# atoms-ufrj/atomsmm

Hardware: AMD Instinct MI355X
Metric: ns/day on 100k-atom TIP3P RESPA box; near-nonbonded HBM GB/s vs 8 TB/s peak (higher is better)
Workload: dtype f64

## Files before the change

atomsmm_amd/csrc/abi.hip:

```cpp
#include <algorithm>
#include <cmath>
#include <cstring>
#include <numeric>

#include "amm_ctx.h"
#include "cluster.h"

int amm_pair_setup_grid(amm_ctx *ctx, PairForce *pf);
static bool amm_family_allows_cluster(int family, int flags) {
    const bool tab_family = family == AMM_NEAR_NONE || family == AMM_NEAR_SHIFT || family == AMM_NEAR_FSWITCH || family == AMM_DAMPED || family == AMM_NONBONDED;
    return tab_family && !(flags & (AMM_GROUP_LJ | AMM_GROUP_Q));
}
int amm_bonded_arity(int kind);
int amm_bonded_npar(int kind);

static thread_local std::string g_error;
void amm_set_error(const std::string &msg) { g_error = msg; }

static PairForce *get_pair(amm_ctx *ctx, int id) {
    if (!ctx || id < 0 || id >= (int)ctx->forces.size() || ctx->forces[id].type != AMM_FORCE_PAIR) {
        amm_set_error("invalid pair force id");
        return nullptr;
    }
    return ctx->forces[id].pair;
// ... 1222 lines not shown
            long long c2 = 0;
            if (amm_pair_count_within_impl(ctx, pf->rest, d_pos, r_within, &c2)) return 1;
            c += c2;
        }
    } else if (amm_pair_count_within_impl(ctx, pf, d_pos, r_within, &c)) return 1;
    *count = (int64_t)c;
    return 0;
}

const char *amm_kernel_revision(void) { return amm_kernel_revision_impl(); }

int amm_set_outer_skin(amm_ctx *ctx, double skin_out) {
    ctx->skin_out = skin_out;
    return 0;
}

int amm_set_option(amm_ctx *ctx, const char *name, double value) {
    if (!ctx || !name) {
        amm_set_error("amm_set_option: null argument");
        return 1;
    }
    const std::string k(name);
    const int v = (int)value;
    if (k == "cluster") ctx->opt_cluster = v;
    else if (k == "hybrid") ctx->opt_hybrid = v;
    else if (k == "small_group") ctx->opt_small_group = v;
    else if (k == "mixed_terms") ctx->opt_mixed_terms = v;
    else if (k == "rest_skin_factor") ctx->opt_rest_skin_factor = value;
    else if (k == "tab") ctx->opt_tab = v;
    else if (k == "site_trips") ctx->site_trips = v != 0;
    else if (k == "lanes_per_row") ctx->opt_lpa = v;
    else if (k == "build_parts") ctx->opt_parts = v;
    else if (k == "build_split") ctx->opt_build_split = v;
    else if (k == "unroll") ctx->opt_unroll = v;
    else if (k == "dual_unroll") ctx->opt_dual_unroll = v;
    else if (k == "tab_block") ctx->opt_tab_bs = v;
    else if (k == "tab_dual_block") ctx->opt_tab_dual_bs = v;
    else if (k == "fuse_rows") ctx->opt_fuse_rows = v;
    else if (k == "row_phases") ctx->opt_row_phases = v;
    else if (k == "group_candidates") ctx->opt_group_candidates = v;
    else if (k == "positions_private") ctx->opt_positions_private = v;
    else if (k == "site_tab") ctx->opt_site_tab = v;
    else if (k == "terms_from") ctx->opt_terms_from = v;
    else if (k == "no_term_lanes") ctx->opt_no_term_lanes = v;
    else if (k == "fuse_epilogue") ctx->opt_fuse_epilogue = v;
    else if (k == "comm_timeout") ctx->opt_comm_timeout = value;
    else if (k == "spec_assign") ctx->opt_spec_assign = v;
    else if (k == "chargeless") ctx->opt_chargeless = v;
    else if (k == "state_exchange") ctx->opt_state_exchange = v;
    else {
        amm_set_error("amm_set_option: unknown option '" + k + "'");
        return 1;
    }
    return 0;
}

static const double AMM_BOX_SKIN_KEEP = 0.5;
static const double AMM_BOX_ROWS_GROW = 1.25;

static double grid_room(const amm_ctx *ctx, const CellGrid &g) {
    double room = 1.0e30;
    for (int k = 0; k < 3; ++k) room = std::min(room, 2.0 * ctx->box.L[k] / g.nc[k]);
    return room;
}
static bool grid_differs(const amm_ctx *ctx, const CellGrid &g, double reach) {
    for (int k = 0; k < 3; ++k) {
// ... 228 lines not shown
```

atomsmm_amd/csrc/amm_ctx.h:

```cpp
#pragma once
#include <hip/hip_runtime.h>

#include <cstdint>
#include <string>
#include <vector>

#include "../../include/atomsmm_hip.h"

#define AMM_WAVE 64
#define AMM_MAX_PRE 6
#define AMM_DERIV_LAMBDA 1024
#define AMM_MAX_GROUPS 33

void amm_set_error(const std::string &msg);
#define AMM_HIP(call)                                                                            \
    do {                                                                                         \
        hipError_t e_ = (call);                                                                  \
        if (e_ != hipSuccess) {                                                                  \
            amm_set_error(std::string(#call) + ": " + hipGetErrorString(e_));                    \
            return 1;                                                                            \
        }                                                                                        \
    } while (0)

struct PairTab {
// ... 259 lines not shown
    BondedSet *bs = nullptr;
    double *f0 = nullptr;
    int npre = 0, niter = 0;
    const double *pre_a[AMM_MAX_PRE] = {nullptr}, *pre_b[AMM_MAX_PRE] = {nullptr};
    double pre_coef[AMM_MAX_PRE] = {0};
    int pre_plus[AMM_MAX_PRE] = {0};
    double c1 = 0, d = 0, c2 = 0;
    PairForce *next = nullptr;
    int kind = 0;
    int with_move = 0;
    double dcoef = 0;
};

struct amm_ctx {
    int n = 0;
    int opt_spec_assign = 1;
    int opt_state_exchange = 1;
    int opt_chargeless = 1;
    int opt_fuse_epilogue = 1;
    const EpiPlan *epi_request = nullptr;
    bool epi_done = false;
    long long n_epilogues = 0;
    long long n_state_exchanges = 0;
    std::vector<const double *> own_only;
    long long n_copies_current = 0;
    int opt_cluster = 1;
    int opt_hybrid = 1;
    double opt_rest_skin_factor = 2.0;
    int opt_mixed_terms = 1;
    int opt_small_group = 1;
    bool creating_rest = false;
    int opt_tab = 1;
    int opt_build_split = 0;
    int opt_lpa = 0, opt_parts = 0, opt_unroll = 2, opt_dual_unroll = 2, opt_tab_bs = 0, opt_tab_dual_bs = 0;
    int opt_site_tab = 1;
    CZeroRows zero_rows = CZeroRows{0, nullptr, nullptr, nullptr};
    int opt_positions_private = 0;
    int opt_group_candidates = 1;
    int opt_row_phases = 1;
    int opt_fuse_rows = 1;
    int opt_terms_from = 8192, opt_no_term_lanes = 0;
    ListWatch watched[AMM_MAX_WATCH];
    int n_watched = 0;
    int device = 0;
    hipStream_t stream = nullptr;
    Box box;
    bool has_box = true;
    int rank = 0, world = 1;
    std::vector<ForceObj> forces;
    double *d_x = nullptr, *d_v = nullptr;
    const double *d_mass = nullptr;
    double *slots[AMM_MAX_SLOTS] = {nullptr};
    GroupDef groups[AMM_MAX_GROUPS];
    bool profile = false;
    int profile_only = -1;
    double *d_scratch = nullptr;
    double *d_expr_part = nullptr;
    double *d_fscratch = nullptr;
    ConstraintSet *constraints = nullptr;
    std::vector<MinObj *> minimizers;
    std::vector<ExprDef> exprs;
    std::vector<BathDef> baths;
    IsoDef iso;
    RegDef reg;
    unsigned long long expr_seed = 0, expr_counter = 0;
    double *alt_x = nullptr, *alt_v = nullptr, *alt_f = nullptr;
// ... 120 lines not shown
```

atomsmm_amd/csrc/cluster.hip:

```cpp
#include <algorithm>
#include <cmath>
#include <cstdio>
#include <cstdlib>
#include <cstring>
#include <type_traits>
#include <vector>

#include "amm_ctx.h"
#include "bonded_terms.h"
#include "cluster.h"
#include "device_utils.h"
#include "pair_math.h"
#include "pair_tab.h"

#ifndef AMM_EXP_NOLJ
#define AMM_EXP_NOLJ 0
#endif

__device__ double amm_erfcx_table_dev_c[AMM_ERFCX_NI * AMM_ERFCX_NC];
static bool g_erfcx_uploaded_c[64] = {false};

void amm_cluster_classify(int n, const std::vector<int> &ptr, const std::vector<int> &idx, std::vector<int> &mol_first, std::vector<int> &rest) {
    mol_first.clear();
    rest.clear();
// ... 203 lines not shown
    for (int off = 32; off > 0; off >>= 1) {
        sum += __shfl_xor(sum, off);
        nr += __shfl_xor(nr, off);
        mx = max(mx, __shfl_xor(mx, off));
    }
    if ((threadIdx.x & 63) == 0) {
        sh_part[threadIdx.x >> 6][0] = sum;
        sh_part[threadIdx.x >> 6][1] = mx;
        sh_part[threadIdx.x >> 6][2] = nr;
    }
    __syncthreads();
    if (threadIdx.x == 0) {
        flags[2] = (int)max(max(sh_part[0][1], sh_part[1][1]), max(sh_part[2][1], sh_part[3][1]));
        counters[1] = sh_part[0][0] + sh_part[1][0] + sh_part[2][0] + sh_part[3][0];
        counters[2] = sh_part[0][2] + sh_part[1][2] + sh_part[2][2] + sh_part[3][2];
        if (!count_only) {
            flags[0] = 0;
            flags[AMM_FLAG_FAR] = 0;
            counters[0] += 1;
        }
    }
}

#ifndef CB_WAVES
#define CB_WAVES 5
#endif
#define CB_OCC __attribute__((amdgpu_waves_per_eu(CB_WAVES)))
#ifdef AMM_CBS_TIMING
__device__ unsigned long long g_cbs_t[8];
#define CBS_STAMP(i) do { const unsigned long long now_ = wall_clock64(); if (w == 0 && lane == 0) atomicAdd(&g_cbs_t[i], now_ - t_last); t_last = now_; } while (0)
#else
#define CBS_STAMP(i) do { } while (0)
#endif
template <bool COUNT_ONLY, bool RINT, bool SLICE = false>
__global__ void __launch_bounds__(256) __attribute__((amdgpu_waves_per_eu(SLICE ? 3 : CB_WAVES))) k_cbuild(int c_begin, int c_end, int parts, const int *__restrict__ cell_start,
                                                const float4 *__restrict__ pos4f, CBoxF box, CellGrid g, float rlist, float rnear2, int cap,
                                                int *nl, int *nnb, int *nnb_near, int *flags, unsigned long long *blockstats,
                                                unsigned long long *counters, int *ticket, int force, const int *slice_cells) {
    if (!force && !flags[0]) return;
    __shared__ int s_rstart[4][128];
    __shared__ int s_rpref[4][128];
    __shared__ float s_rshift[4][3][128];
    __shared__ int s_q[4][CB_BATCH][CB_QCAP];
    __shared__ unsigned char s_coarse[4][CB_COARSE];
    const int lane = threadIdx.x & 63, w = threadIdx.x >> 6;
    const int wave = __builtin_amdgcn_readfirstlane((int)((blockIdx.x * blockDim.x + threadIdx.x) >> 6));
    const float FAR = 1.0e9f;
    const float rlist2 = rlist * rlist;
    unsigned long long wsum = 0, wnear = 0;
    int wmax = 0;
    const int first_cell = SLICE ? __builtin_amdgcn_readfirstlane(slice_cells[0]) : 0;
    const int nunits = SLICE ? (__builtin_amdgcn_readfirstlane(slice_cells[1]) - first_cell + 1) * parts : g.ncell * parts;
    int unit = wave;
#ifdef AMM_CBS_TIMING
    unsigned long long t_last = wall_clock64(), t_drain = 0, n_drain = 0;
#endif
    do {
    const int c = unit < nunits ? first_cell + unit / parts : g.ncell, part = unit % parts;
    int a_begin = 0, a_end = 0;
    if (c < g.ncell) {
        const int cb0 = __builtin_amdgcn_readfirstlane(cell_start[c]), cb1 = __builtin_amdgcn_readfirstlane(cell_start[c + 1]);
        const int per = (cb1 - cb0 + parts - 1) / parts;
        a_begin = max(cb0 + part * per, c_begin);
        a_end = min(min(cb0 + (part + 1) * per, cb1), c_end);
    }
    if (a_begin < a_end) {
        const int ncx = g.nc[0], ncy = g.nc[1], ncz = g.nc[2];
        const int cx = c % ncx, cy = (c / ncx) % ncy, cz = c / (ncx * ncy);
        const int nsx = g.nstencil[0], nsy = g.nstencil[1], ne = nsx * nsy * g.nstencil[2];
        int total;
        {
            int ecs[2] = {0, 0}, len[2] = {0, 0}, inc[2];
            float esx[2] = {0.f, 0.f}, esy[2] = {0.f, 0.f}, esz[2] = {0.f, 0.f};
#pragma unroll
            for (int hh = 0; hh < 2; ++hh) {
                const int e = lane + 64 * hh;
                if (e < ne) {
                    const int ox = e % nsx, oy = (e / nsx) % nsy, oz = e / (nsx * nsy);
                    int nz = ncz < 2 * g.h[2] + 1 ? oz : cz - g.h[2] + oz;
                    esz[hh] = nz < 0 ? -box.L[2] : (nz >= ncz ? box.L[2] : 0.f);
                    nz = nz < 0 ? nz + ncz : (nz >= ncz ? nz - ncz : nz);
                    int ny = ncy < 2 * g.h[1] + 1 ? oy : cy - g.h[1] + oy;
                    esy[hh] = ny < 0 ? -box.L[1] : (ny >= ncy ? box.L[1] : 0.f);
                    ny = ny < 0 ? ny + ncy : (ny >= ncy ? ny - ncy : ny);
                    int nx = ncx < 2 * g.h[0] + 1 ? ox : cx - g.h[0] + ox;
                    esx[hh] = nx < 0 ? -box.L[0] : (nx >= ncx ? box.L[0] : 0.f);
                    nx = nx < 0 ? nx + ncx : (nx >= ncx ? nx - ncx : nx);
                    const int cc = (nz * ncy + ny) * ncx + nx;
                    ecs[hh] = cell_start[cc];
                    len[hh] = cell_start[cc + 1] - ecs[hh];
                }
                inc[hh] = len[hh];
                for (int off = 1; off < 64; off <<= 1) {
                    const int v = __shfl_up(inc[hh], off);
                    if (lane >= off) inc[hh] += v;
                }
            }
            const int lower = __builtin_amdgcn_readlane(inc[0], 63);
            total = lower + __builtin_amdgcn_readlane(inc[1], 63);
#pragma unroll
            for (int hh = 0; hh < 2; ++hh) {
                s_rstart[w][lane + 64 * hh] = ecs[hh];
                s_rpref[w][lane + 64 * hh] = (hh ? lower : 0) + inc[hh] - len[hh];
                s_rshift[w][0][lane + 64 * hh] = esx[hh];
                s_rshift[w][1][lane + 64 * hh] = esy[hh];
                s_rshift[w][2][lane + 64 * hh] = esz[hh];
            }
            __builtin_amdgcn_fence(__ATOMIC_RELEASE, "wavefront");
            __builtin_amdgcn_wave_barrier();
            __builtin_amdgcn_fence(__ATOMIC_ACQUIRE, "wavefront");
        }
        int cshift = 3;
        while (((total + 127) >> cshift) > CB_COARSE) ++cshift;
#pragma unroll
        for (int q = 0; q < CB_COARSE / 64; ++q) {
            const int idx = (lane + 64 * q) << cshift;
            int r = 0;
#pragma unroll
            for (int step = 64; step > 0; step >>= 1)
                if (s_rpref[w][r + step] <= idx) r += step;
            s_coarse[w][lane + 64 * q] = (unsigned char)r;
        }
        __builtin_amdgcn_fence(__ATOMIC_RELEASE, "wavefront");
        __builtin_amdgcn_wave_barrier();
        __builtin_amdgcn_fence(__ATOMIC_ACQUIRE, "wavefront");
#ifdef AMM_CBS_TIMING
        if (SLICE && lane == 0) { atomicAdd(&g_cbs_t[7], 1ull); atomicAdd(&g_cbs_t[0], wall_clock64() - t_last); }
#endif
        for (int tb = a_begin; tb < a_end; tb += CB_BATCH) {
            const int nt = min(CB_BATCH, a_end - tb);
            float4 my = make_float4(0.f, 0.f, 0.f, 0.f);
            if (lane < 3 * nt) my = pos4f[3 * tb + lane];
            int row_cnt = 0;
            int q_head = 0, q_cnt = 0;
            auto rl = [&](float v, int l) { return __int_as_float(__builtin_amdgcn_readlane(__float_as_int(v), l)); };
            auto drain = [&](int t, int n) {
#ifdef AMM_CBS_TIMING
                const unsigned long long t_d0 = wall_clock64();
                n_drain++;
#endif
                const int head = __builtin_amdgcn_readlane(q_head, t);
                int slot[2];
                bool v[2];
                float4 A[2][3];
#pragma unroll
                for (int u = 0; u < 2; ++u) {
                    const bool v0 = lane + 64 * u < n;
                    slot[u] = v0 ? s_q[w][t][cq_wrap(head + lane + 64 * u)] : tb + t;
                    v[u] = v0 && slot[u] != tb + t;
                }
#pragma unroll
                for (int u = 0; u < 2; ++u)
#pragma unroll
                    for (int b = 0; b < 3; ++b) A[u][b] = pos4f[3 * slot[u] + b];
                const int sites[2] = {__float_as_int(A[0][1].w), __float_as_int(A[1][1].w)};
                float px[3], py[3], pz[3];
#pragma unroll
                for (int a = 0; a < 3; ++a) {
                    px[a] = rl(my.x, 3 * t + a);
                    py[a] = rl(my.y, 3 * t + a);
                    pz[a] = rl(my.z, 3 * t + a);
                }
                v2f ax[3], ay[3], az[3];
#pragma unroll
                for (int b = 0; b < 3; ++b) {
                    ax[b] = v2f{A[0][b].x, A[1][b].x};
                    ay[b] = v2f{A[0][b].y, A[1][b].y};
                    az[b] = v2f{A[0][b].z, A[1][b].z};
                }
                if (!RINT) {
                    const v2f sx = box.L[0] * __builtin_elementwise_rint((ax[0] - px[0]) * box.invL[0]);
                    const v2f sy = box.L[1] * __builtin_elementwise_rint((ay[0] - py[0]) * box.invL[1]);
                    const v2f sz = box.L[2] * __builtin_elementwise_rint((az[0] - pz[0]) * box.invL[2]);
#pragma unroll
// ... 12 lines not shown
                        if (RINT) {
                            dx -= box.L[0] * __builtin_elementwise_rint(dx * box.invL[0]);
                            dy -= box.L[1] * __builtin_elementwise_rint(dy * box.invL[1]);
                            dz -= box.L[2] * __builtin_elementwise_rint(dz * box.invL[2]);
                        }
                        v2f r2 = dx * dx;
                        r2 = __builtin_elementwise_fma(dy, dy, r2);
                        r2 = __builtin_elementwise_fma(dz, dz, r2);
                        m2 = __builtin_elementwise_min(m2, r2);
                    }
#pragma unroll
                for (int u = 0; u < 2; ++u) {
                    const float m2u = u ? m2.y : m2.x;
                    const bool pass = v[u] && m2u < rlist2;
                    const unsigned long long m_pass = __builtin_amdgcn_ballot_w64(pass);
                    if (m_pass != 0ull) {
                        const bool is_near = pass && m2u < rnear2;
                        const unsigned long long m_near = __builtin_amdgcn_ballot_w64(is_near);
                        const int np_ = __popcll(m_pass), nn_ = __popcll(m_near);
                        const int c2 = __builtin_amdgcn_readlane(row_cnt, t);
                        const int cnt = c2 & 0xffff, cntf = (int)((unsigned)c2 >> 16);
                        if (!COUNT_ONLY) {
                            const int mp = __builtin_amdgcn_mbcnt_hi((unsigned)(m_pass >> 32), __builtin_amdgcn_mbcnt_lo((unsigned)m_pass, 0u));
                            const int mn = __builtin_amdgcn_mbcnt_hi((unsigned)(m_near >> 32), __builtin_amdgcn_mbcnt_lo((unsigned)m_near, 0u));
                            const int pos_near = cnt + mn, pos_far = (cap - 1 - cntf) - (mp - mn);
                            if (cnt + cntf + np_ <= cap) {
                                int *row_out = nl + (size_t)(tb + t - c_begin) * cap;
                                if (pass) row_out[is_near ? pos_near : pos_far] = slot[u] | (sites[u] << 29);
                            }
                        }
                        row_cnt = lane == t ? c2 + nn_ + ((np_ - nn_) << 16) : row_cnt;
                    }
                }
                q_head = lane == t ? cq_wrap(head + n) : q_head;
                q_cnt = lane == t ? q_cnt - n : q_cnt;
#ifdef AMM_CBS_TIMING
                t_drain += wall_clock64() - t_d0;
#endif
            };
            auto fetch = [&](int cb, float4 (&cand)[2], int (&js)[2]) {
#pragma unroll
                for (int u = 0; u < 2; ++u) {
                    const int idx = cb + u * 64 + lane;
                    const bool in = idx < total;
                    int r = s_coarse[w][idx >> cshift];
                    while (r < 127 && s_rpref[w][r + 1] <= idx) ++r;
                    const int slot = in ? s_rstart[w][r] + idx - s_rpref[w][r] : 0;
                    float4 q = pos4f[3 * slot];
                    if (!RINT) {
                        const float sx = s_rshift[w][0][r], sy = s_rshift[w][1][r], sz = s_rshift[w][2][r];
                        q.x = in ? q.x + sx : FAR;
                        q.y = in ? q.y + sy : FAR;
                        q.z = in ? q.z + sz : FAR;
                    } else if (!in) {
                        q.w = -1.0e9f;
                    }
                    cand[u] = q;
                    js[u] = slot;
                }
            };
            float4 cand[2], cand_n[2];
            int js[2], js_n[2];
            fetch(0, cand, js);
            const float plim_l = my.w + rlist;
            for (int cb = 0; cb < total; cb += 128) {
                if (cb + 128 < total) fetch(cb + 128, cand_n, js_n);
                const v2f cx = v2f{cand[0].x, cand[1].x}, cy = v2f{cand[0].y, cand[1].y}, cz = v2f{cand[0].z, cand[1].z};
                const v2f cw = v2f{cand[0].w, cand[1].w};
                for (int t = 0; t < nt; ++t) {
                    const float p0x = rl(my.x, 3 * t), p0y = rl(my.y, 3 * t), p0z = rl(my.z, 3 * t), plim = rl(plim_l, 3 * t);
                    int qn = __builtin_amdgcn_readlane(q_cnt, t);
                    const int head = __builtin_amdgcn_readlane(q_head, t);
                    v2f dx = p0x - cx, dy = p0y - cy, dz = p0z - cz;
                    if (RINT) {
                        dx -= box.L[0] * __builtin_elementwise_rint(dx * box.invL[0]);
                        dy -= box.L[1] * __builtin_elementwise_rint(dy * box.invL[1]);
                        dz -= box.L[2] * __builtin_elementwise_rint(dz * box.invL[2]);
                    }
                    v2f r2 = dx * dx;
                    r2 = __builtin_elementwise_fma(dy, dy, r2);
                    r2 = __builtin_elementwise_fma(dz, dz, r2);
                    const v2f lim = plim + cw;
                    const v2f lim2 = lim * lim;
#pragma unroll
                    for (int u = 0; u < 2; ++u) {
                        const bool pass = (u ? r2.y < lim2.y : r2.x < lim2.x) && (!RINT || (u ? lim.y : lim.x) > 0.f);
                        const unsigned long long m = __builtin_amdgcn_ballot_w64(pass);
                        if (m == 0ull) continue;
                        const int at = qn + __builtin_amdgcn_mbcnt_hi((unsigned)(m >> 32), __builtin_amdgcn_mbcnt_lo((unsigned)m, 0u));
                        if (pass) s_q[w][t][cq_wrap(head + at)] = js[u];
                        qn += __popcll(m);
                    }
                    q_cnt = lane == t ? qn : q_cnt;
                    if (qn >= 128) {
                        __builtin_amdgcn_fence(__ATOMIC_RELEASE, "wavefront");
                        __builtin_amdgcn_wave_barrier();
                        __builtin_amdgcn_fence(__ATOMIC_ACQUIRE, "wavefront");
                        drain(t, 128);
                    }
                }
#pragma unroll
                for (int u = 0; u < 2; ++u) {
                    cand[u] = cand_n[u];
                    js[u] = js_n[u];
                }
            }
            __builtin_amdgcn_fence(__ATOMIC_RELEASE, "wavefront");
            __builtin_amdgcn_wave_barrier();
            __builtin_amdgcn_fence(__ATOMIC_ACQUIRE, "wavefront");
            for (int t = 0; t < nt; ++t) {
                const int n = __builtin_amdgcn_readlane(q_cnt, t);
                if (n > 0) drain(t, n);
            }
            __builtin_amdgcn_fence(__ATOMIC_RELEASE, "wavefront");
            __builtin_amdgcn_wave_barrier();
            if (lane < nt) {
                const int count = row_cnt & 0xffff, countf = (int)((unsigned)row_cnt >> 16);
                const int total_nb = count + countf;
                if (!COUNT_ONLY) {
                    const bool over = total_nb > cap;
                    nnb[tb + lane - c_begin] = over ? 0 : total_nb;
                    nnb_near[tb + lane - c_begin] = over ? 0 : count;
                    if (over) flags[1] = 1;
                }
                wsum += (unsigned long long)total_nb;
                wnear += (unsigned long long)count;
                wmax = max(wmax, total_nb);
            }
        }
    }
#ifdef AMM_CBS_TIMING
    if (SLICE && lane == 0 && a_begin < a_end) { atomicAdd(&g_cbs_t[1], wall_clock64() - t_last); atomicAdd(&g_cbs_t[2], t_drain); atomicAdd(&g_cbs_t[3], n_drain); }
#endif
    unit += (int)(gridDim.x * (blockDim.x >> 6));
    } while (SLICE && unit < nunits);
    for (int off = 32; off > 0; off >>= 1) {
        wsum += __shfl_xor(wsum, off);
        wnear += __shfl_xor(wnear, off);
        wmax = max(wmax, __shfl_xor(wmax, off));
    }
    __shared__ unsigned long long s_sum[4], s_near[4];
    __shared__ int s_max[4];
    if (lane == 0) {
        s_sum[w] = wsum;
        s_near[w] = wnear;
        s_max[w] = wmax;
    }
    __syncthreads();
    if (threadIdx.x == 0) {
        amm_st_l2(&blockstats[3 * blockIdx.x], s_sum[0] + s_sum[1] + s_sum[2] + s_sum[3]);
        amm_st_l2(&blockstats[3 * blockIdx.x + 1], (unsigned long long)max(max(s_max[0], s_max[1]), max(s_max[2], s_max[3])));
        amm_st_l2(&blockstats[3 * blockIdx.x + 2], s_near[0] + s_near[1] + s_near[2] + s_near[3]);
    }
    if (amm_last_block(ticket)) cfinish_build_block(flags, counters, blockstats, (int)gridDim.x, COUNT_ONLY ? 1 : 0);
}

#ifndef CBS_BATCH
#define CBS_BATCH 3
#endif
#ifndef CBS_SEG
#define CBS_SEG 384
#endif
#define CBS_MAXCH (4 * CBS_SEG / 128)
template <bool RINT>
__global__ void __launch_bounds__(256) k_cbuild_split(int c_begin, int c_end, int parts, const int *__restrict__ cell_start,
                                                      const float4 *__restrict__ pos4f, CBoxF box, CellGrid g, float rlist, float rnear2, int cap,
                                                      int *nl, int *nnb, int *nnb_near, int *flags, unsigned long long *blockstats,
                                                      unsigned long long *counters, int *ticket, int force, const int *slice_cells) {
    if (!force && !flags[0]) return;
    __shared__ int s_rstart[128];
    __shared__ int s_rpref[128];
    __shared__ float s_rshift[3][128];
    __shared__ unsigned char s_coarse[CB_COARSE];
    __shared__ int s_total;
    __shared__ int s_ring[4][CBS_BATCH][CBS_SEG];
    __shared__ int s_cnt[4][CBS_BATCH];
    __shared__ int s_stage[CBS_BATCH * CBS_MAXCH][128];
    __shared__ int s_ccnt[CBS_BATCH * CBS_MAXCH];
    const int lane = threadIdx.x & 63, w = threadIdx.x >> 6;
    const float FAR = 1.0e9f;
    const float rlist2 = rlist * rlist;
    unsigned long long wsum = 0, wnear = 0;
    int wmax = 0;
    const int first_cell = __builtin_amdgcn_readfirstlane(slice_cells[0]);
    const int nunits = (__builtin_amdgcn_readfirstlane(slice_cells[1]) - first_cell + 1) * parts;
    for (int unit = (int)blockIdx.x; unit < nunits; unit += (int)gridDim.x) {
    const int c = first_cell + unit / parts, part = unit % parts;
// ... 1222 lines not shown
        if (nc > 512) nc = 512;
        g.nc[k] = nc;
        g.h[k] = 2;
        g.nstencil[k] = nc >= 5 ? 5 : nc;
        g.cw[k] = L / nc;
        g.inv_cw[k] = nc / L;
        g.ncell *= nc;
        if (!(rc + cl->skin + 2.0 * cl->rext < 0.5 * L * (1 - 1e-9))) cl->per_pair_image = true;
    }
    return 0;
}

static int cluster_chain(amm_ctx *ctx, PairForce *L, ClusterList *cl, const double *d_pos, int force, bool count_only, PairForce *gather_for,
                         CZeroRows Z = CZeroRows{0, nullptr, nullptr, nullptr}, int copies_current = 0, bool skip_assign = false) {
    hipStream_t st = ctx->stream;
    const int nc = cl->nc;
    if (!skip_assign)
        hipLaunchKernelGGL(k_cassign, dim3((nc + cl->nrest + 255) / 256), dim3(256), 0, st, nc, d_pos, ctx->box, cl->grid, cl->d_cell_count, cl->d_cell_start,
                           cl->d_cell_members, cl->capc, count_only ? (double *)nullptr : cl->d_xref, cl->d_flags, cl->d_ticket, force, cl->d_first,
                           cl->d_rest, cl->nrest);
    if (!cl->d_cell_members) return 0;
    PairForce *gf = gather_for;
    const long sort_threads = std::max(std::max((long)cl->grid.ncell * 64, gf ? (long)nc : 0L), (long)Z.n);
    hipLaunchKernelGGL(k_csort_gather, dim3((unsigned)((sort_threads + 255) / 256)), dim3(256), 0, st, cl->grid.ncell, nc, cl->d_cell_start,
                       cl->d_cell_members, cl->capc, cl->d_cperm, cl->d_aperm, d_pos, ctx->box, cl->d_pos4f, cl->d_flags, cl->d_flags, force,
                       gf ? gf->d_q : nullptr, gf ? gf->d_hsig : nullptr, gf ? gf->d_seps2 : nullptr, gf ? gf->d_posq_s : (double4 *)nullptr,
                       gf ? gf->d_lj_s : (double2 *)nullptr, (float)cl->rext, L->d_seps2, cl->d_first, Z, copies_current,
                       count_only ? (double *)nullptr : cl->d_xref, cl->c_begin, cl->c_end, cl->d_slice_cells);
    const bool slice = cl->c_end - cl->c_begin < cl->nc;
    const bool split = cl->split_parts > 0 && !count_only;
    const int ncell_grid = slice ? (int)std::min<long>(cl->grid.ncell, (5L * cl->grid.ncell) / (4L * std::max(1, ctx->world)) + 4) : cl->grid.ncell;
    const long threads = (long)ncell_grid * cl->parts * 64;
    dim3 grid(split ? (unsigned)(ncell_grid * cl->split_parts) : (unsigned)((threads + 255) / 256));
    CBoxF bf;
    for (int k = 0; k < 3; ++k) {
        bf.L[k] = (float)ctx->box.L[k];
        bf.invL[k] = (float)ctx->box.invL[k];
    }
    const float rl = (float)cl->rlist_build;
    const float rn2 = cl->rnear_build > 0 ? (float)(cl->rnear_build * cl->rnear_build) : 3.0e38f;
    const bool use_rint = cl->grid.nc[0] < 5 || cl->grid.nc[1] < 5 || cl->grid.nc[2] < 5;
#define AMM_LAUNCH_CBUILD(CO, RI)                                                                                                   \
    do {                                                                                                                            \
        if (slice)                                                                                                                  \
            hipLaunchKernelGGL((k_cbuild<CO, RI, true>), grid, dim3(256), 0, st, cl->c_begin, cl->c_end, cl->parts, cl->d_cell_start,    \
                               cl->d_pos4f, bf, cl->grid, rl, rn2, cl->cap, cl->d_nl, cl->d_nnb, cl->d_nnb_near, cl->d_flags,            \
                               cl->d_blockstats, cl->d_counters, cl->d_ticket + AMM_TICKET_INTS, force, cl->d_slice_cells);              \
        else                                                                                                                        \
            hipLaunchKernelGGL((k_cbuild<CO, RI, false>), grid, dim3(256), 0, st, cl->c_begin, cl->c_end, cl->parts, cl->d_cell_start,   \
                               cl->d_pos4f, bf, cl->grid, rl, rn2, cl->cap, cl->d_nl, cl->d_nnb, cl->d_nnb_near, cl->d_flags,            \
                               cl->d_blockstats, cl->d_counters, cl->d_ticket + AMM_TICKET_INTS, force, cl->d_slice_cells);              \
    } while (0)
#define AMM_LAUNCH_CBUILD_SPLIT(RI)                                                                                                  \
    hipLaunchKernelGGL((k_cbuild_split<RI>), grid, dim3(256), 0, st, cl->c_begin, cl->c_end, cl->split_parts, cl->d_cell_start,     \
                       cl->d_pos4f, bf, cl->grid, rl, rn2, cl->cap, cl->d_nl, cl->d_nnb, cl->d_nnb_near, cl->d_flags, cl->d_blockstats,  \
                       cl->d_counters, cl->d_ticket + AMM_TICKET_INTS, force, cl->d_slice_cells)
    if (count_only) {
        if (use_rint) AMM_LAUNCH_CBUILD(true, true);
        else AMM_LAUNCH_CBUILD(true, false);
    } else if (split) {
        if (use_rint) AMM_LAUNCH_CBUILD_SPLIT(true);
        else AMM_LAUNCH_CBUILD_SPLIT(false);
    } else {
        if (use_rint) AMM_LAUNCH_CBUILD(false, true);
        else AMM_LAUNCH_CBUILD(false, false);
    }
#undef AMM_LAUNCH_CBUILD
#undef AMM_LAUNCH_CBUILD_SPLIT
    AMM_HIP(hipGetLastError());
    return 0;
}

static double cluster_extent_host(amm_ctx *ctx, const double *d_pos, int n, int nc, const std::vector<int> &first) {
    std::vector<double> x(3 * (size_t)n);
    if (hipMemcpyAsync(x.data(), d_pos, sizeof(double) * 3 * (size_t)n, hipMemcpyDeviceToHost, ctx->stream) != hipSuccess) return -1.0;
    if (hipStreamSynchronize(ctx->stream) != hipSuccess) return -1.0;
    double worst = 0.0;
    for (int m = 0; m < nc; ++m) {
        const size_t i0 = first.empty() ? 3 * (size_t)m : (size_t)first[m];
        for (int a = 1; a < 3; ++a) {
            double d2 = 0.0;
            for (int k = 0; k < 3; ++k) {
                double d = x[3 * (i0 + a) + k] - x[3 * i0 + k];
                d -= ctx->box.L[k] * std::nearbyint(d * ctx->box.invL[k]);
// ... 540 lines not shown
        slots = 64ull * (unsigned long long)longest;
    }
    for (int off = 32; off > 0; off >>= 1) {
        slots += __shfl_xor(slots, off);
        entries += __shfl_xor(entries, off);
    }
    if ((threadIdx.x & 63) == 0) {
        atomicAdd(&out[0], slots);
        atomicAdd(&out[1], entries);
    }
}

int amm_cluster_row_padding_impl(amm_ctx *ctx, PairForce *pf, long long out[2]) {
    PairForce *L = pf->host ? pf->host : pf;
    ClusterList *cl = L->cl;
    hipStream_t st = ctx->stream;
    const int nrows = cl->c_end - cl->c_begin;
    int sh = 0;
    while ((1 << sh) < cl->lpa) ++sh;
    unsigned long long *d_out = cl->d_counters + 5;
    AMM_HIP(hipMemsetAsync(d_out, 0, 2 * sizeof(unsigned long long), st));
    const int ntask = (nrows + (64 >> sh) - 1) / (64 >> sh);
    if (ntask > 0)
        hipLaunchKernelGGL(k_crow_padding, dim3((unsigned)((ntask + 255) / 256)), dim3(256), 0, st, nrows, sh, (pf == L) ? cl->d_nnb : cl->d_nnb_near, d_out);
    unsigned long long h[2] = {0, 0};
    AMM_HIP(hipMemcpyAsync(h, d_out, sizeof(h), hipMemcpyDeviceToHost, st));
    AMM_HIP(hipStreamSynchronize(st));
    out[0] = (long long)h[0];
    out[1] = (long long)h[1];
    return 0;
}

int amm_cluster_free(ClusterList *cl) {
#ifdef AMM_CBS_TIMING
    {
        unsigned long long t[8];
        const bool got = hipMemcpyFromSymbol(t, HIP_SYMBOL(g_cbs_t), sizeof(t)) == hipSuccess && t[7];
        if (got && cl->split_parts == 0)
            fprintf(stderr, "k_cbuild<SLICE>: %llu busy wavefronts, mean: prologue %.2f us, whole %.2f us, in drains %.2f us (%.2f drains)\n", t[7], t[0] / 100.0 / t[7],
                    t[1] / 100.0 / t[7], t[2] / 100.0 / t[7], (double)t[3] / t[7]);
        if (got && cl->split_parts > 0)
            fprintf(stderr, "k_cbuild_split, first wavefront of %llu busy blocks, mean clocks (100 MHz): prologue %.2f | pass 1 %.2f wait %.2f | pass 2 %.2f wait %.2f | copy %.2f wait %.2f us\n",
                    t[7], t[0] / 100.0 / t[7], t[1] / 100.0 / t[7], t[2] / 100.0 / t[7], t[3] / 100.0 / t[7], t[4] / 100.0 / t[7], t[5] / 100.0 / t[7], t[6] / 100.0 / t[7]);
    }
#endif
    for (void *q : {(void *)cl->d_spec_count[0], (void *)cl->d_spec_count[1], (void *)cl->d_spec_ticket})
        if (q) (void)hipFree(q);
    if (cl->d_slice_cells) (void)hipFree(cl->d_slice_cells);
    void *ptrs[] = {cl->d_cell_count, cl->d_cell_start, cl->d_cell_members, cl->d_cperm, cl->d_aperm, cl->d_pos4f, cl->d_xref, cl->d_nl,
                    cl->d_nnb, cl->d_nnb_near, cl->d_flags, cl->d_counters, cl->d_blockstats, cl->d_ticket};
    for (void *p : ptrs)
        if (p) (void)hipFree(p);
    delete cl;
    return 0;
}
```

atomsmm_amd/csrc/pair.hip:

```cpp
#include <atomic>
#include <cmath>
#include <cstdio>
#include <cstdlib>
#include <cstring>

#include "amm_ctx.h"
#include "bonded_terms.h"
#include "cluster.h"
#include "device_utils.h"
#include "pair_math.h"
#include "pair_tab.h"

int amm_pair_build_consts(const amm_pair_desc &d, PairConsts &pc) {
    pc.family = d.family;
    pc.flags = d.flags;
    pc.degree = d.degree < 1 ? 1 : d.degree;
    pc.cmode = (d.flags & AMM_COULOMB_EWALD) ? 1 : ((d.flags & AMM_COULOMB_RF) ? 2 : 0);
    pc.sign = d.sign;
    pc.rc = d.rc;
    pc.rc2 = d.rc * d.rc;
    pc.rc0 = d.rc0;
    pc.rs0 = d.rs0;
    pc.inv_dr0 = (d.rc0 > d.rs0) ? 1.0 / (d.rc0 - d.rs0) : 0.0;
    pc.rswitch = d.rswitch;
// ... 1948 lines not shown
        amm_set_error("amm_pair_count_within: evaluate the force once first (the neighbour rows do not exist yet)");
        return 1;
    }
    hipStream_t st = ctx->stream;
    const int n = pf->n;
    hipLaunchKernelGGL(k_gather_sorted, dim3((n + 255) / 256), dim3(256), 0, st, n, L->d_perm, d_pos, pf->d_q, pf->d_hsig,
                       pf->d_seps2, ctx->box, pf->d_posq_s, pf->d_lj_s);
    PairArgs A;
    std::memset(&A, 0, sizeof(A));
    A.s_begin = L->s_begin;
    A.s_end = L->s_end;
    A.lpa_shift = 3;
    A.cap = L->cap;
    A.nl = L->d_nl;
    A.nnb = L->d_nnb_near;
    A.nnb_total = (pf == L && L->rnear_build > 0) ? L->d_nnb : nullptr;
    A.posq_s = pf->d_posq_s;
    A.box = ctx->box;
    const int nslice = L->s_end - L->s_begin;
    unsigned long long *d_cnt = L->d_counters + 7;
    AMM_HIP(hipMemsetAsync(d_cnt, 0, sizeof(unsigned long long), st));
    if (nslice > 0)
        hipLaunchKernelGGL(k_count_within, dim3((unsigned)(((long)nslice * 8 + 255) / 256)), dim3(256), 0, st, A, r_within * r_within, nslice, d_cnt);
    unsigned long long h = 0;
    AMM_HIP(hipMemcpyAsync(&h, d_cnt, sizeof(h), hipMemcpyDeviceToHost, st));
    AMM_HIP(hipStreamSynchronize(st));
    *count = (long long)h;
    return 0;
}

extern "C" __attribute__((weak)) const char *amm_variant_tag(void);
const char *amm_kernel_revision_impl() {
#ifdef AMM_CLUSTER_TUNE
    return "r06-prologue-tune";
#else
    return amm_variant_tag ? "r06-prologue-tune" : "r06-prologue";
#endif
}

int amm_pair_build_table(PairForce *pf) {
    std::vector<double> coef;
    SiteTable ss;
    ss.want = pf->cluster_ok && pf->one_site_class && pf->site_one_charge && pf->site_q != 0.0 && pf->site_seps2 != 0.0;
    ss.sig = 2.0 * pf->site_hsig;
    ss.eps4 = pf->site_seps2 * pf->site_seps2;
    ss.QQ = pf->pc.Kc * pf->site_q * pf->site_q;
    pf->tab_error = amm_build_coulomb_table(pf->pc, coef, &ss);
    pf->ss_built_for[0] = pf->site_hsig;
    pf->ss_built_for[1] = pf->site_seps2;
    pf->ss_built_for[2] = ss.want ? pf->site_q : 0.0;
    if (pf->d_tab) {
        (void)hipFree(pf->d_tab);
        pf->d_tab = nullptr;
    }
    if (pf->d_tab_ss) {
        (void)hipFree(pf->d_tab_ss);
        pf->d_tab_ss = nullptr;
    }
    pf->ss_error = ss.error;
    static std::atomic<unsigned long long> uploads{0};
    pf->tab_serial = ++uploads;
    if (pf->pc.tab.nint > 0 && !(pf->tab_error <= AMM_TAB_MAX_ERROR)) {
        pf->pc.tab.nint = 0;
        coef.clear();
    }
    if (pf->pc.tab.nint == 0 || ss.coef.empty() || !(ss.error <= AMM_TAB_SS_MAX_ERROR)) {
        pf->pc.tab.ss_first = -1;
        ss.coef.clear();
    }
// ... 87 lines not shown
```

Measured before the change: 1097.

## Schedule cluster-list build work units dynamically with a persistent wave grid

The non-slice neighbor-list build kernel now launches at most a resident-sized grid (CUs times waves per EU). Each wavefront draws cell/part work units from a global atomic counter, grabbing runs of CB_RUN*parts units that other waves in the block can share through an LDS run descriptor. This replaces the one-unit-per-wave static mapping. The goal is to smooth load imbalance and tail effects across uneven cells. It also moves per-wave statistics into LDS atomics and reloads grid geometry and pointers from LDS to cut scalar register pressure. The cost is added atomics and a counter that the last block must reset.

```diff
diff --git a/atomsmm_amd/csrc/abi.hip b/atomsmm_amd/csrc/abi.hip
--- a/atomsmm_amd/csrc/abi.hip
+++ b/atomsmm_amd/csrc/abi.hip
@@ -1278,6 +1278,7 @@
     else if (k == "lanes_per_row") ctx->opt_lpa = v;
     else if (k == "build_parts") ctx->opt_parts = v;
     else if (k == "build_split") ctx->opt_build_split = v;
+    else if (k == "build_dynamic") ctx->opt_build_dynamic = v;
     else if (k == "unroll") ctx->opt_unroll = v;
     else if (k == "dual_unroll") ctx->opt_dual_unroll = v;
     else if (k == "tab_block") ctx->opt_tab_bs = v;
diff --git a/atomsmm_amd/csrc/amm_ctx.h b/atomsmm_amd/csrc/amm_ctx.h
--- a/atomsmm_amd/csrc/amm_ctx.h
+++ b/atomsmm_amd/csrc/amm_ctx.h
@@ -315,6 +315,7 @@
     bool creating_rest = false;
     int opt_tab = 1;
     int opt_build_split = 0;
+    int opt_build_dynamic = 1;
     int opt_lpa = 0, opt_parts = 0, opt_unroll = 2, opt_dual_unroll = 2, opt_tab_bs = 0, opt_tab_dual_bs = 0;
     int opt_site_tab = 1;
     CZeroRows zero_rows = CZeroRows{0, nullptr, nullptr, nullptr};
diff --git a/atomsmm_amd/csrc/cluster.hip b/atomsmm_amd/csrc/cluster.hip
--- a/atomsmm_amd/csrc/cluster.hip
+++ b/atomsmm_amd/csrc/cluster.hip
@@ -259,42 +259,121 @@
 #else
 #define CBS_STAMP(i) do { } while (0)
 #endif
+#ifdef AMM_CB_WAVE_TIMING
+__device__ unsigned long long g_cbw_t[8] = {0, 0, 0, 0, 0, ~0ull, 0, 0};
+#endif
+#ifndef CB_RUN
+#define CB_RUN 4
+#endif
 template <bool COUNT_ONLY, bool RINT, bool SLICE = false>
 __global__ void __launch_bounds__(256) __attribute__((amdgpu_waves_per_eu(SLICE ? 3 : CB_WAVES))) k_cbuild(int c_begin, int c_end, int parts, const int *__restrict__ cell_start,
                                                 const float4 *__restrict__ pos4f, CBoxF box, CellGrid g, float rlist, float rnear2, int cap,
                                                 int *nl, int *nnb, int *nnb_near, int *flags, unsigned long long *blockstats,
-                                                unsigned long long *counters, int *ticket, int force, const int *slice_cells) {
+                                                unsigned long long *counters, int *ticket, int force, const int *slice_cells,
+                                                int *unit_counter) {
     if (!force && !flags[0]) return;
+    const bool dyn = !SLICE && unit_counter != nullptr;
+    __shared__ int s_run;
     __shared__ int s_rstart[4][128];
     __shared__ int s_rpref[4][128];
     __shared__ float s_rshift[4][3][128];
     __shared__ int s_q[4][CB_BATCH][CB_QCAP];
     __shared__ unsigned char s_coarse[4][CB_COARSE];
-    const int lane = threadIdx.x & 63, w = threadIdx.x >> 6;
+    int lane = threadIdx.x & 63, w = threadIdx.x >> 6;
     const int wave = __builtin_amdgcn_readfirstlane((int)((blockIdx.x * blockDim.x + threadIdx.x) >> 6));
     const float FAR = 1.0e9f;
     const float rlist2 = rlist * rlist;
-    unsigned long long wsum = 0, wnear = 0;
-    int wmax = 0;
+    __shared__ unsigned long long s_sum[4], s_near[4];
+    __shared__ int s_max[4];
+    if (lane == 0) {
+        s_sum[w] = 0ull;
+        s_near[w] = 0ull;
+        s_max[w] = 0;
+    }
     const int first_cell = SLICE ? __builtin_amdgcn_readfirstlane(slice_cells[0]) : 0;
     const int nunits = SLICE ? (__builtin_amdgcn_readfirstlane(slice_cells[1]) - first_cell + 1) * parts : g.ncell * parts;
-    int unit = wave;
+    __shared__ int s_geo[12];
+    __shared__ const void *s_ptr[4];
+    if (threadIdx.x == 0) {
+        s_ptr[0] = cell_start;
+        s_ptr[1] = blockstats;
+        s_ptr[2] = counters;
+        s_ptr[3] = ticket;
+    }
+    if (threadIdx.x < 3) {
+        s_geo[threadIdx.x] = g.nc[threadIdx.x];
+        s_geo[3 + threadIdx.x] = g.h[threadIdx.x];
+        s_geo[6 + threadIdx.x] = g.nstencil[threadIdx.x];
+    }
+    if (threadIdx.x == 0) s_geo[9] = g.ncell;
+    __syncthreads();
+    const int runlen = CB_RUN * parts;
+    int p_next = 0, p_end = 0, p_base = 0;
+    auto draw = [&](int *counter, bool lds_max, int v) {
+        int got = 0;
+        if (lane == 0) got = lds_max ? atomicMax(counter, v) : atomicAdd(counter, v);
+        return __builtin_amdgcn_readfirstlane(got);
+    };
+    auto next_unit = [&]() {
+        if (CB_RUN == 0) return draw(unit_counter, false, 1);
+        if (p_next < p_end) return p_base + p_next++;
+        const int old = draw(&s_run, false, 1);
+        if ((old >> 8) > 0 && (old & 0xff) < runlen) return ((old >> 8) - 1) * runlen + (old & 0xff);
+        const int r = draw(unit_counter, false, 1);
+        if ((long)r * runlen >= nunits) return nunits;
+        const int before = draw(&s_run, true, ((r + 1) << 8) | 1);
+        if ((before >> 8) > r + 1) {
+            p_base = r * runlen;
+            p_next = 1;
+            p_end = runlen;
+        } else if ((before >> 8) > 0 && (before & 0xff) < runlen) {
+            p_base = ((before >> 8) - 1) * runlen;
+            p_next = before & 0xff;
+            p_end = runlen;
+        }
+        return r * runlen;
+    };
+    if (dyn && CB_RUN > 0) {
+        if (threadIdx.x == 0) s_run = runlen;
+        __syncthreads();
+    }
+    int unit = dyn ? next_unit() : wave;
 #ifdef AMM_CBS_TIMING
     unsigned long long t_last = wall_clock64(), t_drain = 0, n_drain = 0;
 #endif
+#ifdef AMM_CB_WAVE_TIMING
+    const unsigned long long t_w0 = wall_clock64();
+    unsigned long long n_units = 0;
+#endif
     do {
-    const int c = unit < nunits ? first_cell + unit / parts : g.ncell, part = unit % parts;
+    if (!SLICE) asm volatile("" : "+v"(lane), "+v"(w));
+#ifdef AMM_CB_WAVE_TIMING
+    n_units += unit < nunits ? 1 : 0;
+#endif
+    int zo = 0;
+    asm volatile("" : "+s"(zo));
+    auto geo = [&](int k) { return __builtin_amdgcn_readfirstlane(s_geo[zo + k]); };
+    auto ptr_of = [&](int k) {
+        const unsigned long long v = (unsigned long long)s_ptr[zo + k];
+        return (unsigned long long)(unsigned)__builtin_amdgcn_readfirstlane((int)(unsigned)v) |
+               ((unsigned long long)(unsigned)__builtin_amdgcn_readfirstlane((int)(unsigned)(v >> 32)) << 32);
+    };
+    const int *__restrict__ cstart = (const int *)ptr_of(0);
+    const int g_ncell = geo(9);
+    const int c = unit < nunits ? first_cell + unit / parts : g_ncell, part = unit % parts;
     int a_begin = 0, a_end = 0;
-    if (c < g.ncell) {
-        const int cb0 = __builtin_amdgcn_readfirstlane(cell_start[c]), cb1 = __builtin_amdgcn_readfirstlane(cell_start[c + 1]);
+    if (c < g_ncell) {
+        const int cb0 = __builtin_amdgcn_readfirstlane(cstart[c]), cb1 = __builtin_amdgcn_readfirstlane(cstart[c + 1]);
         const int per = (cb1 - cb0 + parts - 1) / parts;
         a_begin = max(cb0 + part * per, c_begin);
         a_end = min(min(cb0 + (part + 1) * per, cb1), c_end);
     }
     if (a_begin < a_end) {
-        const int ncx = g.nc[0], ncy = g.nc[1], ncz = g.nc[2];
+        const int ncx = geo(0), ncy = geo(1), ncz = geo(2);
+        const int g_h[3] = {geo(3), geo(4), geo(5)};
+        const int g_ns[3] = {geo(6), geo(7), geo(8)};
         const int cx = c % ncx, cy = (c / ncx) % ncy, cz = c / (ncx * ncy);
-        const int nsx = g.nstencil[0], nsy = g.nstencil[1], ne = nsx * nsy * g.nstencil[2];
+        const int nsx = g_ns[0], nsy = g_ns[1], ne = nsx * nsy * g_ns[2];
         int total;
         {
             int ecs[2] = {0, 0}, len[2] = {0, 0}, inc[2];
@@ -304,18 +383,18 @@
                 const int e = lane + 64 * hh;
                 if (e < ne) {
                     const int ox = e % nsx, oy = (e / nsx) % nsy, oz = e / (nsx * nsy);
-                    int nz = ncz < 2 * g.h[2] + 1 ? oz : cz - g.h[2] + oz;
+                    int nz = ncz < 2 * g_h[2] + 1 ? oz : cz - g_h[2] + oz;
                     esz[hh] = nz < 0 ? -box.L[2] : (nz >= ncz ? box.L[2] : 0.f);
                     nz = nz < 0 ? nz + ncz : (nz >= ncz ? nz - ncz : nz);
-                    int ny = ncy < 2 * g.h[1] + 1 ? oy : cy - g.h[1] + oy;
+                    int ny = ncy < 2 * g_h[1] + 1 ? oy : cy - g_h[1] + oy;
                     esy[hh] = ny < 0 ? -box.L[1] : (ny >= ncy ? box.L[1] : 0.f);
                     ny = ny < 0 ? ny + ncy : (ny >= ncy ? ny - ncy : ny);
-                    int nx = ncx < 2 * g.h[0] + 1 ? ox : cx - g.h[0] + ox;
+                    int nx = ncx < 2 * g_h[0] + 1 ? ox : cx - g_h[0] + ox;
                     esx[hh] = nx < 0 ? -box.L[0] : (nx >= ncx ? box.L[0] : 0.f);
                     nx = nx < 0 ? nx + ncx : (nx >= ncx ? nx - ncx : nx);
                     const int cc = (nz * ncy + ny) * ncx + nx;
-                    ecs[hh] = cell_start[cc];
-                    len[hh] = cell_start[cc + 1] - ecs[hh];
+                    ecs[hh] = cstart[cc];
+                    len[hh] = cstart[cc + 1] - ecs[hh];
                 }
                 inc[hh] = len[hh];
                 for (int off = 1; off < 64; off <<= 1) {
@@ -359,14 +438,15 @@
             float4 my = make_float4(0.f, 0.f, 0.f, 0.f);
             if (lane < 3 * nt) my = pos4f[3 * tb + lane];
             int row_cnt = 0;
-            int q_head = 0, q_cnt = 0;
+            int q_hc = 0;
             auto rl = [&](float v, int l) { return __int_as_float(__builtin_amdgcn_readlane(__float_as_int(v), l)); };
             auto drain = [&](int t, int n) {
 #ifdef AMM_CBS_TIMING
                 const unsigned long long t_d0 = wall_clock64();
                 n_drain++;
 #endif
-                const int head = __builtin_amdgcn_readlane(q_head, t);
+                const int hc = __builtin_amdgcn_readlane(q_hc, t);
+                const int head = hc & 0xffff;
                 int slot[2];
                 bool v[2];
                 float4 A[2][3];
@@ -445,8 +525,7 @@
                         row_cnt = lane == t ? c2 + nn_ + ((np_ - nn_) << 16) : row_cnt;
                     }
                 }
-                q_head = lane == t ? cq_wrap(head + n) : q_head;
-                q_cnt = lane == t ? q_cnt - n : q_cnt;
+                q_hc = lane == t ? (cq_wrap(head + n) | (((hc >> 16) - n) << 16)) : q_hc;
 #ifdef AMM_CBS_TIMING
                 t_drain += wall_clock64() - t_d0;
 #endif
@@ -482,8 +561,9 @@
                 const v2f cw = v2f{cand[0].w, cand[1].w};
                 for (int t = 0; t < nt; ++t) {
                     const float p0x = rl(my.x, 3 * t), p0y = rl(my.y, 3 * t), p0z = rl(my.z, 3 * t), plim = rl(plim_l, 3 * t);
-                    int qn = __builtin_amdgcn_readlane(q_cnt, t);
-                    const int head = __builtin_amdgcn_readlane(q_head, t);
+                    const int hc1 = __builtin_amdgcn_readlane(q_hc, t);
+                    int qn = hc1 >> 16;
+                    const int head = hc1 & 0xffff;
                     v2f dx = p0x - cx, dy = p0y - cy, dz = p0z - cz;
                     if (RINT) {
                         dx -= box.L[0] * __builtin_elementwise_rint(dx * box.invL[0]);
@@ -504,7 +584,7 @@
                         if (pass) s_q[w][t][cq_wrap(head + at)] = js[u];
                         qn += __popcll(m);
                     }
-                    q_cnt = lane == t ? qn : q_cnt;
+                    q_hc = lane == t ? (head | (qn << 16)) : q_hc;
                     if (qn >= 128) {
                         __builtin_amdgcn_fence(__ATOMIC_RELEASE, "wavefront");
                         __builtin_amdgcn_wave_barrier();
@@ -522,7 +602,7 @@
             __builtin_amdgcn_wave_barrier();
             __builtin_amdgcn_fence(__ATOMIC_ACQUIRE, "wavefront");
             for (int t = 0; t < nt; ++t) {
-                const int n = __builtin_amdgcn_readlane(q_cnt, t);
+                const int n = __builtin_amdgcn_readlane(q_hc, t) >> 16;
                 if (n > 0) drain(t, n);
             }
             __builtin_amdgcn_fence(__ATOMIC_RELEASE, "wavefront");
@@ -536,36 +616,56 @@
                     nnb_near[tb + lane - c_begin] = over ? 0 : count;
                     if (over) flags[1] = 1;
                 }
-                wsum += (unsigned long long)total_nb;
-                wnear += (unsigned long long)count;
-                wmax = max(wmax, total_nb);
+                atomicAdd(&s_sum[w], (unsigned long long)total_nb);
+                atomicAdd(&s_near[w], (unsigned long long)count);
+                atomicMax(&s_max[w], total_nb);
             }
         }
     }
 #ifdef AMM_CBS_TIMING
     if (SLICE && lane == 0 && a_begin < a_end) { atomicAdd(&g_cbs_t[1], wall_clock64() - t_last); atomicAdd(&g_cbs_t[2], t_drain); atomicAdd(&g_cbs_t[3], n_drain); }
 #endif
-    unit += (int)(gridDim.x * (blockDim.x >> 6));
-    } while (SLICE && unit < nunits);
-    for (int off = 32; off > 0; off >>= 1) {
-        wsum += __shfl_xor(wsum, off);
-        wnear += __shfl_xor(wnear, off);
-        wmax = max(wmax, __shfl_xor(wmax, off));
-    }
-    __shared__ unsigned long long s_sum[4], s_near[4];
-    __shared__ int s_max[4];
-    if (lane == 0) {
-        s_sum[w] = wsum;
-        s_near[w] = wnear;
-        s_max[w] = wmax;
-    }
+    unit = dyn ? next_unit() : unit + (int)(gridDim.x * (blockDim.x >> 6));
+    } while ((SLICE || dyn) && unit < nunits);
+#ifdef AMM_CB_WAVE_TIMING
+    const unsigned long long t_w1 = wall_clock64();
+#endif
     __syncthreads();
+    int zt = 0;
+    asm volatile("" : "+s"(zt));
+    unsigned long long *const bstats = (unsigned long long *)s_ptr[zt + 1];
+    unsigned long long *const cnts = (unsigned long long *)s_ptr[zt + 2];
+    int *const tick = (int *)s_ptr[zt + 3];
     if (threadIdx.x == 0) {
-        amm_st_l2(&blockstats[3 * blockIdx.x], s_sum[0] + s_sum[1] + s_sum[2] + s_sum[3]);
-        amm_st_l2(&blockstats[3 * blockIdx.x + 1], (unsigned long long)max(max(s_max[0], s_max[1]), max(s_max[2], s_max[3])));
-        amm_st_l2(&blockstats[3 * blockIdx.x + 2], s_near[0] + s_near[1] + s_near[2] + s_near[3]);
-    }
-    if (amm_last_block(ticket)) cfinish_build_block(flags, counters, blockstats, (int)gridDim.x, COUNT_ONLY ? 1 : 0);
+        amm_st_l2(&bstats[3 * blockIdx.x], s_sum[0] + s_sum[1] + s_sum[2] + s_sum[3]);
+        amm_st_l2(&bstats[3 * blockIdx.x + 1], (unsigned long long)max(max(s_max[0], s_max[1]), max(s_max[2], s_max[3])));
+        amm_st_l2(&bstats[3 * blockIdx.x + 2], s_near[0] + s_near[1] + s_near[2] + s_near[3]);
+    }
+#ifdef AMM_CB_WAVE_TIMING
+    if (!SLICE && !COUNT_ONLY) {
+        const unsigned long long t_w2 = wall_clock64();
+        if (lane == 0) {
+            atomicAdd(&g_cbw_t[0], t_w1 - t_w0);
+            atomicAdd(&g_cbw_t[1], t_w2 - t_w1);
+            atomicAdd(&g_cbw_t[2], 1ull);
+            atomicAdd(&g_cbw_t[7], n_units);
+            atomicMin(&g_cbw_t[5], t_w0);
+            atomicMax(&g_cbw_t[6], t_w2);
+        }
+    }
+#endif
+    if (amm_last_block(tick)) {
+        if (dyn && threadIdx.x == 0) amm_st_l2(unit_counter, 0);
+#ifdef AMM_CB_WAVE_TIMING
+        if (!SLICE && !COUNT_ONLY && threadIdx.x == 0) {
+            g_cbw_t[3] += 1;
+            g_cbw_t[4] += atomicMax(&g_cbw_t[6], 0ull) - atomicMin(&g_cbw_t[5], ~0ull);
+            __hip_atomic_store(&g_cbw_t[5], ~0ull, __ATOMIC_RELAXED, __HIP_MEMORY_SCOPE_AGENT);
+            __hip_atomic_store(&g_cbw_t[6], 0ull, __ATOMIC_RELAXED, __HIP_MEMORY_SCOPE_AGENT);
+        }
+#endif
+        cfinish_build_block(flags, cnts, bstats, (int)gridDim.x, COUNT_ONLY ? 1 : 0);
+    }
 }
 
 #ifndef CBS_BATCH
@@ -1854,6 +1954,15 @@
     const int ncell_grid = slice ? (int)std::min<long>(cl->grid.ncell, (5L * cl->grid.ncell) / (4L * std::max(1, ctx->world)) + 4) : cl->grid.ncell;
     const long threads = (long)ncell_grid * cl->parts * 64;
     dim3 grid(split ? (unsigned)(ncell_grid * cl->split_parts) : (unsigned)((threads + 255) / 256));
+    int *unit_counter = nullptr;
+    if (!slice && ctx->opt_build_dynamic != 0) {
+        int &ncu = g_num_cu_c[ctx->device & 63];
+        if (!ncu) AMM_HIP(hipDeviceGetAttribute(&ncu, hipDeviceAttributeMultiprocessorCount, ctx->device));
+        const unsigned resident = (unsigned)std::max(1, ncu) * CB_WAVES;
+        const unsigned most = ctx->opt_build_dynamic < 0 ? (unsigned)(-ctx->opt_build_dynamic) : resident;
+        grid.x = std::max(1u, std::min(grid.x, std::min(resident, most)));
+        unit_counter = cl->d_ticket + 2 * AMM_TICKET_INTS;
+    }
     CBoxF bf;
     for (int k = 0; k < 3; ++k) {
         bf.L[k] = (float)ctx->box.L[k];
@@ -1867,11 +1976,13 @@
         if (slice)                                                                                                                  \
             hipLaunchKernelGGL((k_cbuild<CO, RI, true>), grid, dim3(256), 0, st, cl->c_begin, cl->c_end, cl->parts, cl->d_cell_start,    \
                                cl->d_pos4f, bf, cl->grid, rl, rn2, cl->cap, cl->d_nl, cl->d_nnb, cl->d_nnb_near, cl->d_flags,            \
-                               cl->d_blockstats, cl->d_counters, cl->d_ticket + AMM_TICKET_INTS, force, cl->d_slice_cells);              \
+                               cl->d_blockstats, cl->d_counters, cl->d_ticket + AMM_TICKET_INTS, force, cl->d_slice_cells,               \
+                               (int *)nullptr);                                                                                         \
         else                                                                                                                        \
             hipLaunchKernelGGL((k_cbuild<CO, RI, false>), grid, dim3(256), 0, st, cl->c_begin, cl->c_end, cl->parts, cl->d_cell_start,   \
                                cl->d_pos4f, bf, cl->grid, rl, rn2, cl->cap, cl->d_nl, cl->d_nnb, cl->d_nnb_near, cl->d_flags,            \
-                               cl->d_blockstats, cl->d_counters, cl->d_ticket + AMM_TICKET_INTS, force, cl->d_slice_cells);              \
+                               cl->d_blockstats, cl->d_counters, cl->d_ticket + AMM_TICKET_INTS, force, cl->d_slice_cells,               \
+                               unit_counter);                                                                                           \
     } while (0)
 #define AMM_LAUNCH_CBUILD_SPLIT(RI)                                                                                                  \
     hipLaunchKernelGGL((k_cbuild_split<RI>), grid, dim3(256), 0, st, cl->c_begin, cl->c_end, cl->split_parts, cl->d_cell_start,     \
@@ -2478,6 +2589,19 @@
 }
 
 int amm_cluster_free(ClusterList *cl) {
+#ifdef AMM_CB_WAVE_TIMING
+    {
+        unsigned long long t[8];
+        if (hipMemcpyFromSymbol(t, HIP_SYMBOL(g_cbw_t), sizeof(t)) == hipSuccess && t[3]) {
+            const double span = t[4] / 100.0 / t[3];
+            fprintf(stderr, "k_cbuild wave times: %llu builds, %.1f wavefronts and %.1f units per build, span %.2f us; per wavefront working %.2f us, "
+                    "done and waiting for its block %.2f us; mean wavefronts working %.1f, resident %.1f\n", t[3], (double)t[2] / t[3], (double)t[7] / t[3], span,
+                    t[0] / 100.0 / t[2], t[1] / 100.0 / t[2], t[0] / 100.0 / t[3] / span, (t[0] + t[1]) / 100.0 / t[3] / span);
+            const unsigned long long zero[8] = {0, 0, 0, 0, 0, ~0ull, 0, 0};
+            (void)hipMemcpyToSymbol(HIP_SYMBOL(g_cbw_t), zero, sizeof(zero));
+        }
+    }
+#endif
 #ifdef AMM_CBS_TIMING
     {
         unsigned long long t[8];
diff --git a/atomsmm_amd/csrc/pair.hip b/atomsmm_amd/csrc/pair.hip
--- a/atomsmm_amd/csrc/pair.hip
+++ b/atomsmm_amd/csrc/pair.hip
@@ -2004,9 +2004,9 @@
 extern "C" __attribute__((weak)) const char *amm_variant_tag(void);
 const char *amm_kernel_revision_impl() {
 #ifdef AMM_CLUSTER_TUNE
-    return "r06-prologue-tune";
+    return "r07-build-units-tune";
 #else
-    return amm_variant_tag ? "r06-prologue-tune" : "r06-prologue";
+    return amm_variant_tag ? "r07-build-units-tune" : "r07-build-units";
 #endif
 }
 
```

Result: slower. 580.6 (-47.1%).
